# dRaniwal/RAJNI-ViT

Hardware: AMD Instinct MI355X
Metric: images/sec ViT-B/16@224 with README schedule (higher is better)
Workload: dtype bf16

## Files before the change

### rajni-vit_amd/csrc/gemm.hip

```cpp
#include <stdlib.h>
#include <type_traits>
#include "common.h"

namespace {

enum { EPI_BIAS = 0, EPI_GELU = 1, EPI_RESID = 2, EPI_PATCH = 3,
       EPI_GELU8 = 4 };
enum { ALOAD_PLAIN = 0, ALOAD_PATCH = 1 };

struct GemmParams {
  const void* X; long lda;
  const void* W; long ldw;
  const float* wscale;
  const float* xscale;
  const float* yscale;
  const float* bias;
  const float* gamma;
  const void* R; long ldr;
  const int* ridx; int r_np, r_nsrc;
  void* Y; long ldc;
  int M, N, K;
  int tiles_n, total_tiles;
  int nblk;
  int cin, S, log2ps, gw, npatch;
// ... 78 lines not shown
template <bool NT>
__device__ __forceinline__ void store_u4(void* ptr, const uint4& v) {
  if constexpr (NT) __builtin_nontemporal_store(u32x4{v.x, v.y, v.z, v.w}, reinterpret_cast<u32x4*>(ptr));
  else *reinterpret_cast<uint4*>(ptr) = v;
}

template <int EPI, bool SF32, typename A>
__device__ __forceinline__ void epilogue_row(const GemmParams& p, int m, int nbA, int nbB, float* v, const float* gam) {
  long orow = m;
  const bool full = nbB + 8 <= p.N;
  if (EPI == EPI_GELU) {
#pragma unroll
    for (int j = 0; j < 16; j += 4) {
      f32x2 a = f32x2{v[j], v[j + 1]}, b = f32x2{v[j + 2], v[j + 3]};
      gelu_pk4(a, b);
      v[j] = a[0]; v[j + 1] = a[1]; v[j + 2] = b[0]; v[j + 3] = b[1];
    }
  } else if (EPI == EPI_RESID) {
    long rrow = m;
    if (p.ridx != nullptr) {
      const int b = m / p.r_np;
      rrow = (long)b * p.r_nsrc + p.ridx[m];
    }
    const long rbase = rrow * p.ldr;
    if (full) {
      float rf[16];
      load8s<SF32, A>(p.R, rbase + nbA, rf);
      load8s<SF32, A>(p.R, rbase + nbB, rf + 8);
#pragma unroll
      for (int j = 0; j < 16; ++j) v[j] = fmaf(gam[j], v[j], rf[j]);
    } else {
#pragma unroll
      for (int j = 0; j < 16; ++j) {
        const int n = (j < 8 ? nbA : nbB - 8) + j;
        if (n < p.N) v[j] = fmaf(gam[j], v[j], load1<SF32, A>(p.R, rbase + n));
      }
    }
  } else if (EPI == EPI_PATCH) {
    const int b = m / p.npatch, pp = m - b * p.npatch;
    orow = (long)b * (p.npatch + p.nprefix) + p.nprefix + pp;
    const A* pr = reinterpret_cast<const A*>(p.pos) + (long)(pp + p.pos_off) * p.ldc;
    if (full) {
      float pf[16];
      unpack8<A>(*reinterpret_cast<const uint4*>(pr + nbA), pf);
      unpack8<A>(*reinterpret_cast<const uint4*>(pr + nbB), pf + 8);
#pragma unroll
      for (int j = 0; j < 16; ++j) v[j] += pf[j];
    } else {
#pragma unroll
      for (int j = 0; j < 16; ++j) {
        const int n = (j < 8 ? nbA : nbB - 8) + j;
        if (n < p.N) v[j] += ld1(pr + n);
      }
    }
  }
  constexpr bool OUT32 = SF32 && (EPI == EPI_RESID || EPI == EPI_PATCH);
  const long ybase = orow * p.ldc;
  if (full) {
    store8s<OUT32, A>(p.Y, ybase + nbA, v);
    store8s<OUT32, A>(p.Y, ybase + nbB, v + 8);
  } else {
#pragma unroll
    for (int j = 0; j < 16; ++j) {
      const int n = (j < 8 ? nbA : nbB - 8) + j;
      if (n < p.N) store1<OUT32, A>(p.Y, ybase + n, v[j]);
    }
  }
}

constexpr bool nat_order(int epi, bool sf32) { return sf32 && (epi == EPI_RESID || epi == EPI_PATCH); }

enum { MAP_NAT = 1, MAP_SEC = 2, MAP_F8 = 3 };
constexpr int col_map(int epi, bool sf32) { return epi == EPI_GELU8 ? MAP_F8 : nat_order(epi, sf32) ? MAP_NAT : MAP_SEC; }

#ifndef RAJNI_TSTORE
#define RAJNI_TSTORE 1
#endif
#ifndef RAJNI_F8W_LINES
#define RAJNI_F8W_LINES 1
#endif
constexpr bool resid_nat(int epi, bool sf32) { return nat_order(epi, sf32) && epi == EPI_RESID; }
constexpr bool epi_rowmajor(int epi, bool sf32, int mi) { return resid_nat(epi, sf32) && mi <= 4; }
constexpr bool epi_rowmajor_wide(int epi, bool sf32, int mi, bool w8) { return resid_nat(epi, sf32) && mi > 4 && !w8; }
constexpr bool epi_tstore(int epi) { return RAJNI_TSTORE && (epi == EPI_BIAS || epi == EPI_GELU); }
constexpr int stream_scratch_bytes(int epi, bool sf32, int mi, bool w8) {
  return (epi_rowmajor(epi, sf32, mi) || epi_rowmajor_wide(epi, sf32, mi, w8) || epi_tstore(epi)) ? 2048 : 0;
}
constexpr int f8_scratch_bytes(int epi, bool sf32) {
  return (resid_nat(epi, sf32) || epi == EPI_BIAS) ? 2048 : 0;
}
constexpr int f8w_scratch_bytes(int epi) { return (epi == EPI_BIAS && RAJNI_F8W_LINES) ? 4096 : 0; }
constexpr int LDS_MAX_BYTES = 160 * 1024;

template <int MAP>
__device__ __forceinline__ int out_col(int n0w, int g, int j) {
  const int ni = j >> 2, rg = j & 3;
  return MAP == MAP_NAT ? n0w + 16 * ni + 4 * g + rg
       : MAP == MAP_F8 ? n0w + 16 * g + 4 * ni + rg : n0w + 32 * (ni >> 1) + 8 * g + 4 * (ni & 1) + rg;
}
template <int MAP>
__device__ __forceinline__ int w_frag_row(int l15, int ni) {
  return MAP == MAP_NAT ? ni * 16 + l15
       : MAP == MAP_F8 ? 16 * (l15 >> 2) + 4 * ni + (l15 & 3) : 32 * (ni >> 1) + 8 * (l15 >> 2) + 4 * (ni & 1) + (l15 & 3);
}
template <int MAP>
__device__ __forceinline__ int w_key(int row) {
  return MAP == MAP_NAT ? (row >> 1) & 7
       : MAP == MAP_F8 ? ((row >> 4) & 3) * 2 + ((row >> 1) & 1) : ((row >> 3) & 3) * 2 + ((row >> 1) & 1);
}

template <int MAP>
__device__ __forceinline__ int w_key8(int row) {
  return MAP == MAP_NAT ? (row >> 2) & 3 : (row >> 3) & 3;
}
__device__ __forceinline__ bf16x8 fp8x8_to_bf16(uint2 raw) {
  const bf16x2 a = __builtin_amdgcn_cvt_scalef32_pk_bf16_fp8(raw.x, 1.0f, false);
  const bf16x2 b = __builtin_amdgcn_cvt_scalef32_pk_bf16_fp8(raw.x, 1.0f, true);
  const bf16x2 c = __builtin_amdgcn_cvt_scalef32_pk_bf16_fp8(raw.y, 1.0f, false);
  const bf16x2 d = __builtin_amdgcn_cvt_scalef32_pk_bf16_fp8(raw.y, 1.0f, true);
  return bf16x8{a[0], a[1], b[0], b[1], c[0], c[1], d[0], d[1]};
}
typedef __attribute__((ext_vector_type(4))) __bf16 fp8x8_raw;
template <bool W8> struct WFragT { typedef bf16x8 type; };
template <> struct WFragT<true> { typedef fp8x8_raw type; };
__device__ __forceinline__ bf16x8 w_frag_bf16(const bf16x8& f) { return f; }
__device__ __forceinline__ bf16x8 w_frag_bf16(const fp8x8_raw& f) { return fp8x8_to_bf16(__builtin_bit_cast(uint2, f)); }

template <int EPI, typename A>
__device__ __forceinline__ void epilogue_row_nat(const GemmParams& p, int m, int n0w, int g, float* v, const float* gam) {
  long orow = m, rrow = m;
  int pp = 0;
  if (EPI == EPI_RESID && p.ridx != nullptr) {
    const int b = m / p.r_np;
    rrow = (long)b * p.r_nsrc + p.ridx[m];
  }
  if (EPI == EPI_PATCH) {
    const int b = m / p.npatch;
    pp = m - b * p.npatch;
    orow = (long)b * (p.npatch + p.nprefix) + p.nprefix + pp;
  }
  const float* R = reinterpret_cast<const float*>(p.R);
  const A* P = reinterpret_cast<const A*>(p.pos);
  float* Y = reinterpret_cast<float*>(p.Y);
#pragma unroll
  for (int ni = 0; ni < 4; ++ni) {
    const int c = n0w + 16 * ni + 4 * g;
    float* vv = v + 4 * ni;
    if (c + 4 <= p.N) {
      if (EPI == EPI_RESID) {
        const float4 r = *reinterpret_cast<const float4*>(R + rrow * p.ldr + c);
        vv[0] = fmaf(gam[4 * ni + 0], vv[0], r.x); vv[1] = fmaf(gam[4 * ni + 1], vv[1], r.y);
        vv[2] = fmaf(gam[4 * ni + 2], vv[2], r.z); vv[3] = fmaf(gam[4 * ni + 3], vv[3], r.w);
      } else {
        const uint2 q = *reinterpret_cast<const uint2*>(P + (long)(pp + p.pos_off) * p.ldc + c);
        vv[0] += lo16<A>(q.x); vv[1] += hi16<A>(q.x); vv[2] += lo16<A>(q.y); vv[3] += hi16<A>(q.y);
      }
      *reinterpret_cast<float4*>(Y + orow * p.ldc + c) = make_float4(vv[0], vv[1], vv[2], vv[3]);
    } else {
#pragma unroll
      for (int e = 0; e < 4; ++e)
        if (c + e < p.N) {
          float o = vv[e];
          if (EPI == EPI_RESID) o = fmaf(gam[4 * ni + e], o, R[rrow * p.ldr + c + e]);
          else o += ld1(P + (long)(pp + p.pos_off) * p.ldc + c + e);
          Y[orow * p.ldc + c + e] = o;
          vv[e] = o;
// ... 48 lines not shown
                                               int l15, int g) {
  pre.valid = false;
  if constexpr (nat_order(EPI, SF32) && EPI == EPI_RESID && MI <= 4) {
    if (n0w + 64 <= p.N && m_base + MI * 16 <= p.M) {
      const float* R = reinterpret_cast<const float*>(p.R);
#pragma unroll
      for (int mi = 0; mi < MI; ++mi) {
        const int m = m_base + mi * 16 + l15;
        long rrow = m;
        if (p.ridx != nullptr) rrow = (long)(m / p.r_np) * p.r_nsrc + p.ridx[m];
#pragma unroll
        for (int ni = 0; ni < 4; ++ni)
          pre.r[mi][ni] = *reinterpret_cast<const float4*>(R + rrow * p.ldr + n0w + 16 * ni + 4 * g);
      }
      pre.valid = true;
    }
  }
}

constexpr int stores_acc_layout(bool nat, int mi) { return (nat ? 4 : 2) * mi; }
constexpr int stores_rowmajor(int mi) { return 2 * 2 * mi; }
constexpr int stores_tstore(int mi) { return 2 * mi; }
constexpr int tile_stores(int epi, bool sf32, int mi, bool rowmajor, bool tstore) {
  int n = stores_acc_layout(nat_order(epi, sf32), mi);
  if (rowmajor && stores_rowmajor(mi) < n) n = stores_rowmajor(mi);
  if (tstore && stores_tstore(mi) < n) n = stores_tstore(mi);
  return n;
}

template <typename A, int EPI, bool SF32, int MI, bool W8 = false>
__device__ __forceinline__ void epilogue_tile(const GemmParams& p, f32x4 (&acc)[4][MI], int m_base, int n0w,
                                              int l15, int g, ResidPrefetch<MI>& pre, int m_lo = 0,
                                              bool interior = false, char* scratch = nullptr) {
  constexpr int MAP = col_map(EPI, SF32);
  constexpr bool NAT = MAP == MAP_NAT;
  if constexpr (NAT && EPI == EPI_RESID && MI <= 4) {
    if (scratch != nullptr && pre.valid) {
      int lane = g * 16 + l15;
      asm volatile("" : "+v"(lane));
      const int rr = lane >> 3, cc = lane & 7;
      float bias[2][4], gam[2][4], wsc[2][W8 ? 4 : 1];
#pragma unroll
      for (int hc = 0; hc < 2; ++hc) {
        const int n = n0w + 32 * hc + 4 * cc;
        const float4 bq = p.bias != nullptr ? *reinterpret_cast<const float4*>(p.bias + n) : make_float4(0.f, 0.f, 0.f, 0.f);
        const float4 gq = p.gamma != nullptr ? *reinterpret_cast<const float4*>(p.gamma + n) : make_float4(1.f, 1.f, 1.f, 1.f);
        bias[hc][0] = bq.x; bias[hc][1] = bq.y; bias[hc][2] = bq.z; bias[hc][3] = bq.w;
        gam[hc][0] = gq.x; gam[hc][1] = gq.y; gam[hc][2] = gq.z; gam[hc][3] = gq.w;
        if constexpr (W8) {
          const float4 wq = *reinterpret_cast<const float4*>(p.wscale + n);
          wsc[hc][0] = wq.x; wsc[hc][1] = wq.y; wsc[hc][2] = wq.z; wsc[hc][3] = wq.w;
        }
      }
      __builtin_amdgcn_s_waitcnt(0x0F70);
      float* Y = reinterpret_cast<float*>(p.Y) + n0w + 4 * cc;
#pragma unroll
      for (int mi = 0; mi < MI; ++mi)
#pragma unroll
        for (int hc = 0; hc < 2; ++hc) {
#pragma unroll
          for (int q = 0; q < 2; ++q) {
            const int slot = (4 * q + g) ^ (l15 & 7);
            *reinterpret_cast<bf16x8*>(scratch + l15 * 128 + slot * 16) = __builtin_bit_cast(bf16x8, acc[2 * hc + q][mi]);
          }
          __builtin_amdgcn_fence(__ATOMIC_RELEASE, "wavefront");
          __builtin_amdgcn_wave_barrier();
#pragma unroll
          for (int j = 0; j < 2; ++j) {
            const int row = 8 * j + rr, slot = cc ^ (row & 7);
            const f32x4 a = __builtin_bit_cast(f32x4, *reinterpret_cast<const bf16x8*>(scratch + row * 128 + slot * 16));
            const float4 r = pre.r[mi][2 * hc + j];
            float4 o;
            o.x = fmaf(gam[hc][0], W8 ? fmaf(a[0], wsc[hc][0], bias[hc][0]) : a[0] + bias[hc][0], r.x);
            o.y = fmaf(gam[hc][1], W8 ? fmaf(a[1], wsc[hc][1], bias[hc][1]) : a[1] + bias[hc][1], r.y);
            o.z = fmaf(gam[hc][2], W8 ? fmaf(a[2], wsc[hc][2], bias[hc][2]) : a[2] + bias[hc][2], r.z);
            o.w = fmaf(gam[hc][3], W8 ? fmaf(a[3], wsc[hc][3], bias[hc][3]) : a[3] + bias[hc][3], r.w);
            *reinterpret_cast<float4*>(Y + (long)(m_base + mi * 16 + row) * p.ldc + 32 * hc) = o;
          }
          __builtin_amdgcn_wave_barrier();
        }
      return;
    }
  }
  if constexpr (NAT && EPI == EPI_RESID && MI > 4 && !W8) {
    if (scratch != nullptr && interior && p.ridx == nullptr) {
      int lane = g * 16 + l15;
      asm volatile("" : "+v"(lane));
      const int rr = lane >> 3, cc = lane & 7;
      float bias[2][4], gam[2][4];
#pragma unroll
      for (int hc = 0; hc < 2; ++hc) {
        const int n = n0w + 32 * hc + 4 * cc;
        const float4 bq = p.bias != nullptr ? *reinterpret_cast<const float4*>(p.bias + n) : make_float4(0.f, 0.f, 0.f, 0.f);
        const float4 gq = p.gamma != nullptr ? *reinterpret_cast<const float4*>(p.gamma + n) : make_float4(1.f, 1.f, 1.f, 1.f);
        bias[hc][0] = bq.x; bias[hc][1] = bq.y; bias[hc][2] = bq.z; bias[hc][3] = bq.w;
        gam[hc][0] = gq.x; gam[hc][1] = gq.y; gam[hc][2] = gq.z; gam[hc][3] = gq.w;
      }
      const float* R = reinterpret_cast<const float*>(p.R) + n0w + 4 * cc;
      float* Y = reinterpret_cast<float*>(p.Y) + n0w + 4 * cc;
#pragma unroll
      for (int mi = 0; mi < MI; ++mi) {
        float4 r[4];
#pragma unroll
        for (int j = 0; j < 2; ++j) {
          const long ro = (long)(m_base + mi * 16 + 8 * j + rr) * p.ldr;
          r[j] = *reinterpret_cast<const float4*>(R + ro);
          r[2 + j] = *reinterpret_cast<const float4*>(R + ro + 32);
        }
#pragma unroll
        for (int hc = 0; hc < 2; ++hc) {
#pragma unroll
          for (int q = 0; q < 2; ++q) {
            const int slot = (4 * q + g) ^ (l15 & 7);
            *reinterpret_cast<bf16x8*>(scratch + l15 * 128 + slot * 16) = __builtin_bit_cast(bf16x8, acc[2 * hc + q][mi]);
          }
          __builtin_amdgcn_fence(__ATOMIC_RELEASE, "wavefront");
          __builtin_amdgcn_wave_barrier();
#pragma unroll
          for (int j = 0; j < 2; ++j) {
            const int row = 8 * j + rr, slot = cc ^ (row & 7);
            const f32x4 a = __builtin_bit_cast(f32x4, *reinterpret_cast<const bf16x8*>(scratch + row * 128 + slot * 16));
            float4 o;
            o.x = fmaf(gam[hc][0], a[0] + bias[hc][0], r[2 * hc + j].x);
            o.y = fmaf(gam[hc][1], a[1] + bias[hc][1], r[2 * hc + j].y);
            o.z = fmaf(gam[hc][2], a[2] + bias[hc][2], r[2 * hc + j].z);
            o.w = fmaf(gam[hc][3], a[3] + bias[hc][3], r[2 * hc + j].w);
            *reinterpret_cast<float4*>(Y + (long)(m_base + mi * 16 + row) * p.ldc + 32 * hc) = o;
          }
          __builtin_amdgcn_wave_barrier();
        }
      }
      __builtin_amdgcn_s_waitcnt(0x0F70);
      return;
    }
  }
  if constexpr (MAP == MAP_SEC && (EPI == EPI_BIAS || EPI == EPI_GELU)) {
    if (interior) {
      const int ca = n0w + 8 * g, cb = ca + 32;
      float bs[16], ws[16];
#pragma unroll
      for (int j = 0; j < 16; ++j) { bs[j] = 0.f; ws[j] = 1.f; }
      if (p.bias != nullptr) {
        load8<float>(p.bias + ca, bs);
        load8<float>(p.bias + cb, bs + 8);
      }
      if constexpr (W8) {
        load8<float>(p.wscale + ca, ws);
        load8<float>(p.wscale + cb, ws + 8);
      }
      __builtin_amdgcn_s_waitcnt(0x0F70);
      A* Y = reinterpret_cast<A*>(p.Y);
#pragma unroll
      for (int mi = 0; mi < MI; ++mi) {
        float v[16];
#pragma unroll
        for (int j = 0; j < 16; ++j) {
          const int ni = j >> 2, rg = j & 3, o = (ni >> 1) * 8 + (ni & 1) * 4 + rg;
          v[o] = W8 ? fmaf(acc[ni][mi][rg], ws[o], bs[o]) : acc[ni][mi][rg] + bs[o];
        }
        if (EPI == EPI_GELU) {
#pragma unroll
          for (int j = 0; j < 16; j += 4) {
            f32x2 a = f32x2{v[j], v[j + 1]}, b = f32x2{v[j + 2], v[j + 3]};
            gelu_pk4(a, b);
            v[j] = a[0]; v[j + 1] = a[1]; v[j + 2] = b[0]; v[j + 3] = b[1];
          }
        }
        if (scratch != nullptr) {
          int lane = g * 16 + l15;
          asm volatile("" : "+v"(lane));
          const int rr = lane >> 3, cc = lane & 7;
          const int key = l15 & 7;
          *reinterpret_cast<bf16x8*>(scratch + l15 * 128 + ((g ^ key) << 4)) = __builtin_bit_cast(bf16x8, pack8<A>(v));
          *reinterpret_cast<bf16x8*>(scratch + l15 * 128 + (((4 + g) ^ key) << 4)) = __builtin_bit_cast(bf16x8, pack8<A>(v + 8));
          __builtin_amdgcn_fence(__ATOMIC_RELEASE, "wavefront");
          __builtin_amdgcn_wave_barrier();
#pragma unroll
          for (int j = 0; j < 2; ++j) {
            const int row = 8 * j + rr;
            const uint4 q = __builtin_bit_cast(uint4, *reinterpret_cast<const bf16x8*>(scratch + row * 128 + ((cc ^ (row & 7)) << 4)));
            store_u4<RAJNI_FC1_NT && EPI == EPI_GELU>(Y + (long)(m_base + mi * 16 + row) * p.ldc + n0w + 8 * cc, q);
          }
          __builtin_amdgcn_wave_barrier();
        } else {
          A* row = Y + (long)(m_base + mi * 16 + l15) * p.ldc;
          store_u4<RAJNI_FC1_NT && EPI == EPI_GELU>(row + ca, pack8<A>(v));
          store_u4<RAJNI_FC1_NT && EPI == EPI_GELU>(row + cb, pack8<A>(v + 8));
        }
      }
      return;
    }
  }
  float bias[16], gam[16];
#pragma unroll
  for (int j = 0; j < 16; ++j) {
    const int n = out_col<MAP>(n0w, g, j);
    bias[j] = (p.bias != nullptr && n < p.N) ? p.bias[n] : 0.f;
    gam[j] = (EPI == EPI_RESID && p.gamma != nullptr && n < p.N) ? p.gamma[n] : 1.f;
  }
  float wsc[W8 ? 16 : 1];
  if constexpr (W8) {
#pragma unroll
    for (int j = 0; j < 16; ++j) {
      const int n = out_col<MAP>(n0w, g, j);
      wsc[j] = n < p.N ? p.wscale[n] : 0.f;
    }
  }
  __builtin_amdgcn_s_waitcnt(0x0F70);
  auto sb = [&](float a, int j) { return W8 ? fmaf(a, wsc[W8 ? j : 0], bias[j]) : a + bias[j]; };
  if constexpr (NAT && EPI == EPI_RESID && MI <= 4) {
    if (pre.valid) {
      float* Y = reinterpret_cast<float*>(p.Y);
#pragma unroll
      for (int mi = 0; mi < MI; ++mi) {
#pragma unroll
        for (int ni = 0; ni < 4; ++ni) {
          float4 o;
          o.x = fmaf(gam[4 * ni + 0], sb(acc[ni][mi][0], 4 * ni + 0), pre.r[mi][ni].x);
          o.y = fmaf(gam[4 * ni + 1], sb(acc[ni][mi][1], 4 * ni + 1), pre.r[mi][ni].y);
          o.z = fmaf(gam[4 * ni + 2], sb(acc[ni][mi][2], 4 * ni + 2), pre.r[mi][ni].z);
          o.w = fmaf(gam[4 * ni + 3], sb(acc[ni][mi][3], 4 * ni + 3), pre.r[mi][ni].w);
          *reinterpret_cast<float4*>(Y + (long)(m_base + mi * 16 + l15) * p.ldc + n0w + 16 * ni + 4 * g) = o;
        }
      }
      return;
    }
  }
#pragma unroll
  for (int mi = 0; mi < MI; ++mi) {
    const int m = m_base + mi * 16 + l15;
    if (m >= p.M || m < m_lo) continue;
    float v[16];
#pragma unroll
    for (int ni = 0; ni < 4; ++ni)
#pragma unroll
      for (int rg = 0; rg < 4; ++rg) v[ni * 4 + rg] = sb(acc[ni][mi][rg], ni * 4 + rg);
    if (NAT) epilogue_row_nat<EPI, A>(p, m, n0w, g, v, gam);
    else epilogue_row<EPI, SF32, A>(p, m, n0w + 8 * g, n0w + 32 + 8 * g, v, gam);
  }
}
__device__ __forceinline__ int xcd_tile_of(int v, int total) {
  const int q = total >> 3, r = total & 7, xcd = v & 7, loc = v >> 3;
  return (xcd < r ? xcd * (q + 1) : r * (q + 1) + (xcd - r) * q) + loc;
}
__device__ __forceinline__ int xcd_tile(int total) { return xcd_tile_of(blockIdx.x, total); }

template <int ALOAD, typename ET = bf16_t>
struct XSource {
  static constexpr int CH = 16 / (int)sizeof(ET);
  const ET* base;
  int kofs;
  __device__ __forceinline__ void init(const GemmParams& p, int m, int chunk) {
    const ET* X = reinterpret_cast<const ET*>(p.X);
    if (ALOAD == ALOAD_PLAIN) {
      base = X + (long)m * p.lda + chunk * CH;
      kofs = 0;
    } else {
      const int b = m / p.npatch, pp = m - b * p.npatch;
      const int py = pp / p.gw, px = pp - py * p.gw;
      base = X + ((long)b * p.cin * p.S + (py << p.log2ps)) * p.S + (px << p.log2ps);
      kofs = chunk * CH;
    }
  }
  __device__ __forceinline__ const ET* at(const GemmParams& p, int k0) const {
    if (ALOAD == ALOAD_PLAIN) return base + k0;
    const int k = k0 + kofs, ps2 = 2 * p.log2ps;
    const int ch = k >> ps2, rem = k & ((1 << ps2) - 1);
    const int ky = rem >> p.log2ps, kx = rem & ((1 << p.log2ps) - 1);
    return base + ((long)ch * p.S + ky) * p.S + kx;
  }
};

#define RAJNI_GEMM_NBLK_BYTES (1600 * 1024)
namespace wide {
constexpr int BM = 256, BK = 64;
constexpr int X_BYTES = BM * BK * 2;
__device__ __forceinline__ int key_x(int row) { return (row >> 1) & 7; }

template <int WN_, int NS_, bool W8_ = false, int NW_ = 8> struct Cfg {
  static constexpr int BN = WN_ * 64;
  static constexpr int WB = W8_ ? 1 : 2;
  static constexpr int W_BYTES = BN * BK * WB;
  static constexpr int STAGE_BYTES = X_BYTES + W_BYTES;
  static constexpr int LDS_BYTES = NS_ * STAGE_BYTES;
  static constexpr int XP = X_BYTES / 1024 / NW_;
  static constexpr int PW = W_BYTES / 1024 / NW_;
  static constexpr int PIECES = XP + PW;
  static constexpr int NPW = PW < (W8_ ? 2 : 4) ? PW : (W8_ ? 2 : 4);
};
template <int EPI, bool SF32, int WN, int MI, int NS, bool W8>
constexpr int lds_bytes() { return Cfg<WN, NS, W8>::LDS_BYTES + 8 * stream_scratch_bytes(EPI, SF32, MI, W8); }

__host__ __device__ constexpr int dma_first(int g, int pieces, int groups) { return g * pieces / groups; }
__host__ __device__ constexpr int rd_first(int g, int mi, int ni) { return g + g * ni / mi; }
template <int G, int MI, bool DMA, int PIECES, int NI = 4>
__device__ __forceinline__ void sched_half() {
  if constexpr (G < MI) {
    __builtin_amdgcn_sched_group_barrier(0x008, NI, 0);
    if constexpr (rd_first(G + 1, MI, NI) - rd_first(G, MI, NI) > 0)
      __builtin_amdgcn_sched_group_barrier(0x100, rd_first(G + 1, MI, NI) - rd_first(G, MI, NI), 0);
    if constexpr (DMA) {
      constexpr int nd = dma_first(G + 1, PIECES, MI) - dma_first(G, PIECES, MI);
      if constexpr (nd > 0) __builtin_amdgcn_sched_group_barrier(0x020, nd, 0);
    }
    sched_half<G + 1, MI, DMA, PIECES, NI>();
  }
}
template <int N> __device__ __forceinline__ void wait_step() {
  static_assert(N >= 0 && N < 64, "vmcnt is a 6-bit counter");
  asm volatile("s_waitcnt vmcnt(%0) lgkmcnt(0)" :: "n"(N) : "memory");
}

template <int EPI, int ALOAD, bool SF32, int WM, int WN, int MI, int NS, bool W8 = false, int TAG = 0, typename A = bf16_t>
__global__ void __launch_bounds__(WM * WN * 64, 2) gemm_bf16_tn_stream(const GemmParams p) {
  using C = Cfg<WN, NS, W8, WM * WN>;
  constexpr int NI = 4;
  using WFrag = typename WFragT<W8>::type;
  constexpr int MAP = col_map(EPI, SF32);
  static_assert(WM * WN == 8 && WM * MI * 16 == BM, "8 waves covering 256 rows");
  extern __shared__ __attribute__((aligned(16))) char smem[];
  const int tid = threadIdx.x, lane = tid & 63;
  const int wave = __builtin_amdgcn_readfirstlane(tid >> 6);
  constexpr bool ROWMAJOR = epi_rowmajor(EPI, SF32, MI);
  constexpr int SCRATCH = stream_scratch_bytes(EPI, SF32, MI, W8);
  static_assert(lds_bytes<EPI, SF32, WN, MI, NS, W8>() <= LDS_MAX_BYTES, "stages + epilogue scratch exceed the workgroup's LDS");

  auto tile_m0 = [&](int tm_) { return tm_ * BM + BM > p.M ? p.M - BM : tm_ * BM; };
  const int tiles_m = p.total_tiles / p.tiles_n;
  auto tile_mn = [&](int t, int& tm_, int& tn_) {
    if (p.nblk >= p.tiles_n) { tm_ = t / p.tiles_n; tn_ = t - tm_ * p.tiles_n; return; }
    const int per = p.nblk * tiles_m, blk = t / per, r = t - blk * per;
    const int left = p.tiles_n - blk * p.nblk, nb = left < p.nblk ? left : p.nblk;
    const int rr = r / nb;
    tm_ = rr; tn_ = blk * p.nblk + (r - rr * nb);
  };
  XSource<ALOAD> xs[ALOAD == ALOAD_PLAIN ? 1 : C::XP];
  const char* xp[2];
  const char* ws[C::NPW];
  auto point_at = [&](int tile) {
    int tm, tn;
    tile_mn(tile, tm, tn);
    const int r_in = lane >> 3, pch = lane & 7;
    if constexpr (ALOAD == ALOAD_PLAIN) {
#pragma unroll
      for (int i = 0; i < 2; ++i) {
        const int row = (wave * C::XP + i) * 8 + r_in;
        xp[i] = reinterpret_cast<const char*>(p.X) + ((long)(tile_m0(tm) + row) * p.lda + (pch ^ key_x(row)) * 8) * 2;
      }
    } else {
#pragma unroll
      for (int i = 0; i < C::XP; ++i) {
        const int row = (wave * C::XP + i) * 8 + r_in;
        int m = tm * BM + row;
        if (m > p.M - 1) m = p.M - 1;
        xs[i].init(p, m, pch ^ key_x(row));
      }
    }
#pragma unroll
    for (int i = 0; i < C::NPW; ++i) {
      if constexpr (W8) {
        const int row = (wave * C::PW + i) * 16 + (lane >> 2);
        ws[i] = reinterpret_cast<const char*>(p.W) + (long)(tn * C::BN + row) * p.ldw + (((lane & 3) ^ w_key8<MAP>(row)) << 4);
      } else {
        const int row = (wave * C::PW + i) * 8 + r_in;
        ws[i] = reinterpret_cast<const char*>(p.W) + ((long)(tn * C::BN + row) * p.ldw + (pch ^ w_key<MAP>(row)) * 8) * 2;
      }
    }
  };
  auto advance = [&](int from, int to) {
    if constexpr (ALOAD == ALOAD_PLAIN) {
      int tm0, tn0, tm1, tn1;
      tile_mn(from, tm0, tn0);
      tile_mn(to, tm1, tn1);
      const long dx = (long)(tile_m0(tm1) - tile_m0(tm0)) * p.lda * 2;
      const long dw = (long)(tn1 - tn0) * C::BN * p.ldw * C::WB;
      xp[0] += dx; xp[1] += dx;
#pragma unroll
      for (int i = 0; i < C::NPW; ++i) ws[i] += dw;
    } else {
      point_at(to);
    }
  };
  auto dma_piece = [&](int q, int k0, char* dx) {
    if (q < C::XP) {
      if constexpr (ALOAD == ALOAD_PLAIN)
        __builtin_amdgcn_global_load_lds(GLB_PTR(xp[q & 1] + ((long)(q >> 1) * 16 * p.lda + k0) * 2),
                                         LDS_PTR(dx + (wave * C::XP + q) * 1024), 16, 0, 0);
      else
        __builtin_amdgcn_global_load_lds(GLB_PTR(xs[q].at(p, k0)), LDS_PTR(dx + (wave * C::XP + q) * 1024), 16, 0, 0);
    } else {
      const int i = q - C::XP;
      if constexpr (C::PW <= C::NPW)
        __builtin_amdgcn_global_load_lds(GLB_PTR(ws[i] + k0 * C::WB), LDS_PTR(dx + X_BYTES + (wave * C::PW + i) * 1024), 16, 0, 0);
      else
        __builtin_amdgcn_global_load_lds(GLB_PTR(ws[i % C::NPW] + ((long)(i / C::NPW) * 32 * p.ldw + k0) * C::WB),
                                         LDS_PTR(dx + X_BYTES + (wave * C::PW + i) * 1024), 16, 0, 0);
    }
  };
  auto stage = [&](int kt, int st) {
#pragma unroll
    for (int q = 0; q < C::PIECES; ++q) dma_piece(q, kt * BK, smem + st * C::STAGE_BYTES);
  };

  const int wm = wave / WN, wn = wave % WN;
  const int l15 = lane & 15, g = lane >> 4;
  const int xr0 = wm * (MI * 16) + l15;
  const int wr0 = wn * 64 + w_frag_row<MAP>(l15, 0);
  auto w_ni_off = [](int ni) { return (w_frag_row<MAP>(0, ni) - w_frag_row<MAP>(0, 0)) * (64 * C::WB); };
  int xo[2], wo[2];
#pragma unroll
  for (int ks = 0; ks < 2; ++ks) {
    xo[ks] = xr0 * 128 + (((ks * 4 + g) ^ key_x(xr0)) << 4);
    if constexpr (W8)
      wo[ks] = X_BYTES + wr0 * 64 + ((((ks * 4 + g) >> 1) ^ w_key8<MAP>(wr0)) << 4) + ((g & 1) << 3);
    else
      wo[ks] = X_BYTES + wr0 * 128 + (((ks * 4 + g) ^ w_key<MAP>(wr0)) << 4);
  }

  f32x4 acc[4][MI];

  auto half = [&](auto dma_c, auto read_c, bf16x8 (&xc)[MI], WFrag (&wc)[NI], bf16x8 (&xn)[MI], WFrag (&wn_)[NI],
                  int rst, int rks, int dkt, int dst) {
    constexpr bool DMA = decltype(dma_c)::value;
    constexpr bool READ = decltype(read_c)::value;
    const char* sb = smem + rst * C::STAGE_BYTES;
    char* dx = smem + dst * C::STAGE_BYTES;
    const int k0 = dkt * BK;
    bf16x8 wv[NI];
#pragma unroll
    for (int ni = 0; ni < NI; ++ni) wv[ni] = w_frag_bf16(wc[ni]);
#pragma unroll
    for (int mi = 0; mi < MI; ++mi) {
#pragma unroll
      for (int ni = 0; ni < NI; ++ni)
        acc[ni][mi] = mfma_16x16x32<A>(wv[ni], xc[mi], acc[ni][mi]);
      if constexpr (READ) {
        xn[mi] = *reinterpret_cast<const bf16x8*>(sb + xo[rks] + mi * 2048);
#pragma unroll
        for (int wi = mi * NI / MI; wi < (mi + 1) * NI / MI; ++wi)
          wn_[wi] = *reinterpret_cast<const WFrag*>(sb + wo[rks] + w_ni_off(wi));
      }
      if constexpr (DMA) {
#pragma unroll
        for (int q = dma_first(mi, C::PIECES, MI); q < dma_first(mi + 1, C::PIECES, MI); ++q) dma_piece(q, k0, dx);
      }
    }
    if constexpr (READ) sched_half<0, MI, DMA, C::PIECES, NI>();
  };
  using T = std::true_type; using F = std::false_type;
  const int nk = p.K / BK;
  int v = blockIdx.x;
  int tile = xcd_tile_of(v, p.total_tiles);
  bf16x8 xa[MI], xb[MI];
  WFrag wa[NI], wb[NI];
  if constexpr (EPI == EPI_RESID) {
    if (p.stagger > 0 && ((blockIdx.x >> 3) & 1))
      for (int i = 0; i < p.stagger; ++i) __builtin_amdgcn_s_sleep(127);
  }

  constexpr int WBASE = (NS - 2) * C::PIECES;
  auto interior = [&](int t) {
    int tm_, tn_;
    tile_mn(t, tm_, tn_);
    return tm_ * BM + BM <= p.M && tn_ * C::BN + C::BN <= p.N;
  };
  ResidPrefetch<MI> pre;
  point_at(tile);
#pragma unroll
  for (int j = 0; j < NS; ++j) stage(j, j);
  wait_step<((NS - 1) * C::PIECES > 8) ? 0 : (NS - 1) * C::PIECES>();
  __builtin_amdgcn_s_barrier();
  asm volatile("" ::: "memory");
#pragma unroll
  for (int i = 0; i < NI; ++i) wa[i] = *reinterpret_cast<const WFrag*>(smem + wo[0] + w_ni_off(i));
#pragma unroll
  for (int i = 0; i < MI; ++i) xa[i] = *reinterpret_cast<const bf16x8*>(smem + xo[0] + i * 2048);
  int st = 0;
  constexpr int NSTORE_ALL = tile_stores(EPI, SF32, MI, ROWMAJOR || epi_rowmajor_wide(EPI, SF32, MI, W8), epi_tstore(EPI));
  constexpr int NSTORE = NSTORE_ALL < 48 ? NSTORE_ALL : 48;
  bool prev_full = false;

  while (true) {
#ifdef RAJNI_GEMM_STAMPS
    const unsigned long long ts0 = __builtin_amdgcn_s_memtime();
#endif
    int tm, tn;
    tile_mn(tile, tm, tn);
    const int m0 = ALOAD == ALOAD_PLAIN ? tile_m0(tm) : tm * BM, n0 = tn * C::BN;
    const int m_lo = tm * BM;
    const bool inter = interior(tile);
    const int vn = v + gridDim.x;
    const bool more = vn < p.total_tiles;
    pre.valid = false;
#pragma unroll
    for (int a = 0; a < 4; ++a)
#pragma unroll
      for (int b = 0; b < MI; ++b) acc[a][b] = f32x4{0.f, 0.f, 0.f, 0.f};

    auto kstep = [&](int kt) {
      if (kt == nk - NS && more) advance(tile, xcd_tile_of(vn, p.total_tiles));
      const int dkt = kt + NS < nk ? kt + NS : kt + NS - nk;
      const int st1 = st + 1 == NS ? 0 : st + 1;
      if (kt == nk - 1 && inter) {
        if constexpr (ROWMAJOR) prefetch_resid_rowmajor<MI>(p, pre, m0 + wm * (MI * 16), n0 + wn * 64, lane);
        else prefetch_resid<EPI, SF32, MI>(p, pre, m0 + wm * (MI * 16), n0 + wn * 64, l15, g);
      }
      half(F{}, T{}, xa, wa, xb, wb, st, 1, 0, 0);
      if (NSTORE > 0 && kt == 0 && prev_full) wait_step<WBASE + NSTORE>();
      else wait_step<WBASE>();
      __builtin_amdgcn_s_barrier();
      asm volatile("" ::: "memory");
      half(T{}, T{}, xb, wb, xa, wa, st1, 0, dkt, st);
      st = st1;
    };
    for (int kt = 0; kt < nk; ++kt) kstep(kt);
#ifdef RAJNI_GEMM_STAMPS
    asm volatile("" :: "v"(acc[0][0][0]), "v"(acc[3][MI - 1][3]));
    const unsigned long long ts2 = __builtin_amdgcn_s_memtime();
#endif

    epilogue_tile<A, EPI, SF32, MI, W8>(p, acc, m0 + wm * (MI * 16), n0 + wn * 64, l15, g, pre, m_lo, inter,
                                     SCRATCH > 0 ? smem + C::LDS_BYTES + wave * SCRATCH : nullptr);
#ifdef RAJNI_GEMM_STAMPS
    if (p.stamps != nullptr && wave == 0) {
      const unsigned long long ts3 = __builtin_amdgcn_s_memtime();
      if (lane == 0) {
        unsigned long long* o = p.stamps + (size_t)tile * 4;
        o[0] = ts0; o[1] = ts0; o[2] = ts2; o[3] = ts3;
      }
    }
#endif
    prev_full = inter;
    if (!more) break;
    v = vn;
    tile = xcd_tile_of(v, p.total_tiles);
  }
  asm volatile("s_waitcnt vmcnt(0)" ::: "memory");
}
}

namespace small {
constexpr int BM = 128, BN = 128, BK = 64;
constexpr int TILE_BYTES = BM * BK * 2;
constexpr int STAGE_BYTES = 2 * TILE_BYTES;
constexpr int LDS_BYTES = 2 * STAGE_BYTES;
__device__ __forceinline__ int key_x(int row) { return (row >> 1) & 7; }
__device__ __forceinline__ int key_w(int row) { return ((row >> 4) & 3) * 2 + ((row >> 1) & 1); }

template <int EPI, int ALOAD, bool SF32, bool W8 = false, typename A = bf16_t>
__global__ void __launch_bounds__(256, 2) gemm_bf16_tn_128x128(const GemmParams p) {
  constexpr int MAP = col_map(EPI, SF32);
  constexpr int PW = W8 ? 2 : 4;
  using WFrag = typename WFragT<W8>::type;
  extern __shared__ __attribute__((aligned(16))) char smem[];
  const int tid = threadIdx.x, lane = tid & 63;
  const int wave = __builtin_amdgcn_readfirstlane(tid >> 6);
  const int t = xcd_tile(p.total_tiles);
  const int tm = t / p.tiles_n, tn = t - tm * p.tiles_n;
  const int m0 = tm * BM, n0 = tn * BN;

  const int r_in = lane >> 3, pch = lane & 7;
  XSource<ALOAD> xs[4];
  const char* ws[PW];
#pragma unroll
  for (int i = 0; i < 4; ++i) {
    const int row = (wave * 4 + i) * 8 + r_in;
    int m = m0 + row;
    if (m > p.M - 1) m = p.M - 1;
    xs[i].init(p, m, pch ^ key_x(row));
  }
#pragma unroll
  for (int i = 0; i < PW; ++i) {
    if constexpr (W8) {
      const int row = (wave * PW + i) * 16 + (lane >> 2);
      ws[i] = reinterpret_cast<const char*>(p.W) + (long)(n0 + row) * p.ldw + (((lane & 3) ^ w_key8<MAP>(row)) << 4);
    } else {
      const int row = (wave * PW + i) * 8 + r_in;
      ws[i] = reinterpret_cast<const char*>(p.W) + ((long)(n0 + row) * p.ldw + (pch ^ w_key<MAP>(row)) * 8) * 2;
    }
  }
  auto stage = [&](int kt, int buf) {
    char* sx = smem + buf * STAGE_BYTES;
    char* sw = sx + TILE_BYTES;
    const int k0 = kt * BK;
#pragma unroll
    for (int i = 0; i < 4; ++i)
      __builtin_amdgcn_global_load_lds(GLB_PTR(xs[i].at(p, k0)), LDS_PTR(sx + (wave * 4 + i) * 1024), 16, 0, 0);
#pragma unroll
    for (int i = 0; i < PW; ++i)
      __builtin_amdgcn_global_load_lds(GLB_PTR(ws[i] + k0 * (W8 ? 1 : 2)), LDS_PTR(sw + (wave * PW + i) * 1024), 16, 0, 0);
  };

  const int wm = wave >> 1, wn = wave & 1;
  const int l15 = lane & 15, g = lane >> 4;
  int xoff[4], xkey[4], woff[4], wkey[4];
#pragma unroll
  for (int i = 0; i < 4; ++i) {
    const int xr = wm * 64 + i * 16 + l15;
    xoff[i] = xr * 128; xkey[i] = key_x(xr);
    const int wr = wn * 64 + w_frag_row<MAP>(l15, i);
    woff[i] = wr * (W8 ? 64 : 128); wkey[i] = W8 ? w_key8<MAP>(wr) : w_key<MAP>(wr);
  }

  f32x4 acc[4][4];
#pragma unroll
  for (int a = 0; a < 4; ++a)
#pragma unroll
    for (int b = 0; b < 4; ++b) acc[a][b] = f32x4{0.f, 0.f, 0.f, 0.f};

  const int nk = p.K / BK;
  ResidPrefetch<4> pre;
  pre.valid = false;
  stage(0, 0);
  for (int kt = 0; kt < nk; ++kt) {
    asm volatile("s_waitcnt vmcnt(0)" ::: "memory");
    __syncthreads();
    if (kt + 1 < nk) stage(kt + 1, (kt + 1) & 1);
    else prefetch_resid<EPI, SF32, 4>(p, pre, m0 + wm * 64, n0 + wn * 64, l15, g);
// ... 568 lines not shown
```

Measured before the change: 30590.

## Stage residual tiles into LDS via DMA during the last k-steps of the wide resid GEMM

For the wide residual-epilogue GEMM variant, the last two k-steps are peeled. While they run, residual rows are loaded straight into freed LDS stage slots with global_load_lds, and the epilogue then reads them from LDS. The epilogue also refills slots and issues the next tile's operand DMA part-way through, so the residual read and the next tile's loads overlap with compute and stores. This adds complex vmcnt/lgkmcnt bookkeeping and slot-reuse hazards, and keeps a fallback path for non-interior tiles.

```diff
diff --git a/rajni-vit_amd/csrc/gemm.hip b/rajni-vit_amd/csrc/gemm.hip
--- a/rajni-vit_amd/csrc/gemm.hip
+++ b/rajni-vit_amd/csrc/gemm.hip
@@ -398,58 +398,6 @@
       return;
     }
   }
-  if constexpr (NAT && EPI == EPI_RESID && MI > 4 && !W8) {
-    if (scratch != nullptr && interior && p.ridx == nullptr) {
-      int lane = g * 16 + l15;
-      asm volatile("" : "+v"(lane));
-      const int rr = lane >> 3, cc = lane & 7;
-      float bias[2][4], gam[2][4];
-#pragma unroll
-      for (int hc = 0; hc < 2; ++hc) {
-        const int n = n0w + 32 * hc + 4 * cc;
-        const float4 bq = p.bias != nullptr ? *reinterpret_cast<const float4*>(p.bias + n) : make_float4(0.f, 0.f, 0.f, 0.f);
-        const float4 gq = p.gamma != nullptr ? *reinterpret_cast<const float4*>(p.gamma + n) : make_float4(1.f, 1.f, 1.f, 1.f);
-        bias[hc][0] = bq.x; bias[hc][1] = bq.y; bias[hc][2] = bq.z; bias[hc][3] = bq.w;
-        gam[hc][0] = gq.x; gam[hc][1] = gq.y; gam[hc][2] = gq.z; gam[hc][3] = gq.w;
-      }
-      const float* R = reinterpret_cast<const float*>(p.R) + n0w + 4 * cc;
-      float* Y = reinterpret_cast<float*>(p.Y) + n0w + 4 * cc;
-#pragma unroll
-      for (int mi = 0; mi < MI; ++mi) {
-        float4 r[4];
-#pragma unroll
-        for (int j = 0; j < 2; ++j) {
-          const long ro = (long)(m_base + mi * 16 + 8 * j + rr) * p.ldr;
-          r[j] = *reinterpret_cast<const float4*>(R + ro);
-          r[2 + j] = *reinterpret_cast<const float4*>(R + ro + 32);
-        }
-#pragma unroll
-        for (int hc = 0; hc < 2; ++hc) {
-#pragma unroll
-          for (int q = 0; q < 2; ++q) {
-            const int slot = (4 * q + g) ^ (l15 & 7);
-            *reinterpret_cast<bf16x8*>(scratch + l15 * 128 + slot * 16) = __builtin_bit_cast(bf16x8, acc[2 * hc + q][mi]);
-          }
-          __builtin_amdgcn_fence(__ATOMIC_RELEASE, "wavefront");
-          __builtin_amdgcn_wave_barrier();
-#pragma unroll
-          for (int j = 0; j < 2; ++j) {
-            const int row = 8 * j + rr, slot = cc ^ (row & 7);
-            const f32x4 a = __builtin_bit_cast(f32x4, *reinterpret_cast<const bf16x8*>(scratch + row * 128 + slot * 16));
-            float4 o;
-            o.x = fmaf(gam[hc][0], a[0] + bias[hc][0], r[2 * hc + j].x);
-            o.y = fmaf(gam[hc][1], a[1] + bias[hc][1], r[2 * hc + j].y);
-            o.z = fmaf(gam[hc][2], a[2] + bias[hc][2], r[2 * hc + j].z);
-            o.w = fmaf(gam[hc][3], a[3] + bias[hc][3], r[2 * hc + j].w);
-            *reinterpret_cast<float4*>(Y + (long)(m_base + mi * 16 + row) * p.ldc + 32 * hc) = o;
-          }
-          __builtin_amdgcn_wave_barrier();
-        }
-      }
-      __builtin_amdgcn_s_waitcnt(0x0F70);
-      return;
-    }
-  }
   if constexpr (MAP == MAP_SEC && (EPI == EPI_BIAS || EPI == EPI_GELU)) {
     if (interior) {
       const int ca = n0w + 8 * g, cb = ca + 32;
@@ -555,6 +503,76 @@
     else epilogue_row<EPI, SF32, A>(p, m, n0w + 8 * g, n0w + 32 + 8 * g, v, gam);
   }
 }
+__device__ __forceinline__ int lane_now() {
+  unsigned all = ~0u;
+  asm volatile("" : "+s"(all));
+  return (int)__builtin_amdgcn_mbcnt_hi(all, __builtin_amdgcn_mbcnt_lo(all, 0u));
+}
+constexpr int WIDE_LDS_STORES_AFTER_DMA = 4;
+template <int N> __device__ __forceinline__ void wait_vm() {
+  static_assert(N >= 0 && N < 64, "vmcnt is a 6-bit counter");
+  asm volatile("s_waitcnt vmcnt(%0)" :: "n"(N) : "memory");
+}
+__device__ const float WIDE_LDS_ZEROS[4] = {0.f, 0.f, 0.f, 0.f}, WIDE_LDS_ONES[4] = {1.f, 1.f, 1.f, 1.f};
+typedef __attribute__((address_space(1))) f32x4 GLB_F32X4;
+__device__ __forceinline__ unsigned resid_lane_offset(const GemmParams& p, int lane) {
+  return ((unsigned)(lane >> 3) * (unsigned)p.ldr + 4u * (unsigned)(lane & 7)) * 4u;
+}
+__device__ __forceinline__ void land_resid_piece(const GemmParams& p, unsigned lane_off, int m_base, int n0w, int grp, int pc, char* slot) {
+  const char* base = reinterpret_cast<const char*>(p.R) + ((long)(m_base + grp * 16 + (pc & 1) * 8) * p.ldr + n0w + (pc >> 1) * 32) * 4;
+  __builtin_amdgcn_global_load_lds(GLB_PTR(base + (unsigned long)lane_off), LDS_PTR(slot + pc * 1024), 16, 0, 0);
+}
+template <typename SlotFn, typename RefillFn>
+__device__ __forceinline__ void epilogue_wide_lds(const GemmParams& p, f32x4 (&acc)[4][8], int m_base, int n0w,
+                                                  const float (&bias)[2][4], const float (&gam)[2][4], char* scratch,
+                                                  SlotFn&& slot, RefillFn&& refill) {
+  const int lane = lane_now();
+  const int l15 = lane & 15, g = lane >> 4;
+  const int rr = lane >> 3, cc = lane & 7;
+  const unsigned ylo = ((unsigned)rr * (unsigned)p.ldc + 4u * (unsigned)cc) * 4u;
+#pragma unroll
+  for (int mi = 0; mi < 8; ++mi) {
+    if (mi == 0) wait_vm<12>();
+    else if (mi == 1) wait_vm<16>();
+    else if (mi == 2) wait_vm<20>();
+    else if (mi == 3) wait_vm<24>();
+    else wait_vm<28>();
+    const char* sl = slot(mi & 3) + lane * 16;
+    f32x4 r[4];
+#pragma unroll
+    for (int pc = 0; pc < 4; ++pc) r[pc] = __builtin_bit_cast(f32x4, *reinterpret_cast<const bf16x8*>(sl + pc * 1024));
+#pragma unroll
+    for (int hc = 0; hc < 2; ++hc) {
+#pragma unroll
+      for (int q = 0; q < 2; ++q) {
+        const int sw = (4 * q + g) ^ (l15 & 7);
+        *reinterpret_cast<bf16x8*>(scratch + l15 * 128 + sw * 16) = __builtin_bit_cast(bf16x8, acc[2 * hc + q][mi]);
+      }
+      __builtin_amdgcn_fence(__ATOMIC_RELEASE, "wavefront");
+      __builtin_amdgcn_wave_barrier();
+      f32x4 a[2];
+#pragma unroll
+      for (int j = 0; j < 2; ++j) {
+        const int row = 8 * j + rr, sw = cc ^ (row & 7);
+        a[j] = __builtin_bit_cast(f32x4, *reinterpret_cast<const bf16x8*>(scratch + row * 128 + sw * 16));
+      }
+      if (hc == 0) {
+        asm volatile("s_waitcnt lgkmcnt(0)" ::: "memory");
+        refill(mi);
+      }
+#pragma unroll
+      for (int j = 0; j < 2; ++j) {
+        const f32x4 rv = r[2 * hc + j];
+        f32x4 o;
+#pragma unroll
+        for (int e = 0; e < 4; ++e) o[e] = fmaf(gam[hc][e], a[j][e] + bias[hc][e], rv[e]);
+        char* yb = reinterpret_cast<char*>(p.Y) + ((long)(m_base + mi * 16 + 8 * j) * p.ldc + n0w + 32 * hc) * 4;
+        *(GLB_F32X4*)GLB_PTR(yb + (unsigned long)ylo) = o;
+      }
+      __builtin_amdgcn_wave_barrier();
+    }
+  }
+}
 __device__ __forceinline__ int xcd_tile_of(int v, int total) {
   const int q = total >> 3, r = total & 7, xcd = v & 7, loc = v >> 3;
   return (xcd < r ? xcd * (q + 1) : r * (q + 1) + (xcd - r) * q) + loc;
@@ -638,6 +656,8 @@
   const int tid = threadIdx.x, lane = tid & 63;
   const int wave = __builtin_amdgcn_readfirstlane(tid >> 6);
   constexpr bool ROWMAJOR = epi_rowmajor(EPI, SF32, MI);
+  constexpr bool LAND = epi_rowmajor_wide(EPI, SF32, MI, W8);
+  static_assert(!LAND || (NS == 2 && C::XP == 4 && C::PW == 4 && ALOAD == ALOAD_PLAIN), "a slot = the 4 pieces one wave stages of one operand");
   constexpr int SCRATCH = stream_scratch_bytes(EPI, SF32, MI, W8);
   static_assert(lds_bytes<EPI, SF32, WN, MI, NS, W8>() <= LDS_MAX_BYTES, "stages + epilogue scratch exceed the workgroup's LDS");
 
@@ -793,12 +813,22 @@
   for (int i = 0; i < MI; ++i) xa[i] = *reinterpret_cast<const bf16x8*>(smem + xo[0] + i * 2048);
   int st = 0;
   constexpr int NSTORE_ALL = tile_stores(EPI, SF32, MI, ROWMAJOR || epi_rowmajor_wide(EPI, SF32, MI, W8), epi_tstore(EPI));
-  constexpr int NSTORE = NSTORE_ALL < 48 ? NSTORE_ALL : 48;
+  static_assert(!LAND || WIDE_LDS_STORES_AFTER_DMA <= NSTORE_ALL, "the landing epilogue's count must be the smallest of the paths'");
+  constexpr int NSTORE = LAND ? WIDE_LDS_STORES_AFTER_DMA : NSTORE_ALL < 48 ? NSTORE_ALL : 48;
   bool prev_full = false;
 
   while (true) {
 #ifdef RAJNI_GEMM_STAMPS
     const unsigned long long ts0 = __builtin_amdgcn_s_memtime();
+    auto stamp_tile = [&](unsigned long long t0, unsigned long long t2) {
+      if (p.stamps != nullptr && wave == 0) {
+        const unsigned long long ts3 = __builtin_amdgcn_s_memtime();
+        if (lane == 0) {
+          unsigned long long* o = p.stamps + (size_t)tile * 4;
+          o[0] = t0; o[1] = t0; o[2] = t2; o[3] = ts3;
+        }
+      }
+    };
 #endif
     int tm, tn;
     tile_mn(tile, tm, tn);
@@ -829,22 +859,155 @@
       half(T{}, T{}, xb, wb, xa, wa, st1, 0, dkt, st);
       st = st1;
     };
-    for (int kt = 0; kt < nk; ++kt) kstep(kt);
+    [[maybe_unused]] bool landed = false;
+    if constexpr (!LAND) {
+      for (int kt = 0; kt < nk; ++kt) kstep(kt);
+    } else {
+      landed = inter && p.ridx == nullptr && p.ldr < (1L << 26) && p.ldc < (1L << 26);
+      const int nk_main = landed ? nk - 2 : nk;
+      for (int kt = 0; kt < nk_main; ++kt) kstep(kt);
+    }
+    [[maybe_unused]] float lbias[2][4], lgam[2][4];
+    [[maybe_unused]] int st_a = 0;
+    if constexpr (LAND) {
+      if (landed) {
+        const int mw = m0 + wm * (MI * 16), nw = n0 + wn * 64;
+        st_a = st;
+        auto slot = [&](int s) { return smem + ((s >> 1) ? st_a ^ 1 : st_a) * C::STAGE_BYTES + (s & 1) * X_BYTES + wave * 4096; };
+        auto land_piece = [&](unsigned lo, int grp, int pc) { land_resid_piece(p, lo, mw, nw, grp, pc, slot(grp & 3)); };
+        auto half_land = [&](auto read_c, bf16x8 (&xc)[MI], WFrag (&wc)[NI], bf16x8 (&xn)[MI], WFrag (&wn_)[NI], int rst, int grp0) {
+          constexpr bool READ = decltype(read_c)::value;
+          const char* sb = smem + rst * C::STAGE_BYTES;
+          const unsigned lo = resid_lane_offset(p, lane_now());
+          bf16x8 wv[NI];
+#pragma unroll
+          for (int ni = 0; ni < NI; ++ni) wv[ni] = w_frag_bf16(wc[ni]);
+#pragma unroll
+          for (int mi = 0; mi < MI; ++mi) {
+#pragma unroll
+            for (int ni = 0; ni < NI; ++ni)
+              acc[ni][mi] = mfma_16x16x32<A>(wv[ni], xc[mi], acc[ni][mi]);
+            if constexpr (READ) {
+              xn[mi] = *reinterpret_cast<const bf16x8*>(sb + xo[0] + mi * 2048);
+#pragma unroll
+              for (int wi = mi * NI / MI; wi < (mi + 1) * NI / MI; ++wi)
+                wn_[wi] = *reinterpret_cast<const WFrag*>(sb + wo[0] + w_ni_off(wi));
+            }
+            land_piece(lo, grp0 + (mi >> 2), mi & 3);
+          }
+          if constexpr (READ) {
+            sched_half<0, MI, true, C::PIECES, NI>();
+          } else {
+#pragma unroll
+            for (int mi = 0; mi < MI; ++mi) {
+              __builtin_amdgcn_sched_group_barrier(0x008, NI, 0);
+              __builtin_amdgcn_sched_group_barrier(0x020, 1, 0);
+            }
+          }
+        };
+        half(F{}, T{}, xa, wa, xb, wb, st, 1, 0, 0);
+        wait_step<WBASE>();
+        __builtin_amdgcn_s_barrier();
+        asm volatile("" ::: "memory");
+        half_land(T{}, xb, wb, xa, wa, st ^ 1, 0);
+        st ^= 1;
+        half(F{}, T{}, xa, wa, xb, wb, st, 1, 0, 0);
+        asm volatile("s_waitcnt lgkmcnt(0)" ::: "memory");
+        __builtin_amdgcn_s_barrier();
+        asm volatile("" ::: "memory");
+        {
+          const bool hb = p.bias != nullptr, hg = p.gamma != nullptr;
+          const char* bsrc = hb ? reinterpret_cast<const char*>(p.bias + nw) : reinterpret_cast<const char*>(WIDE_LDS_ZEROS);
+          const char* gsrc = hg ? reinterpret_cast<const char*>(p.gamma + nw) : reinterpret_cast<const char*>(WIDE_LDS_ONES);
+          const unsigned lo = 16u * (unsigned)(lane_now() & 7);
+          const unsigned blo = hb ? lo : 0u, glo = hg ? lo : 0u, bhi = hb ? 128u : 0u, ghi = hg ? 128u : 0u;
+#pragma unroll
+          for (int hc = 0; hc < 2; ++hc) {
+            const f32x4 bq = *(const GLB_F32X4*)GLB_PTR(bsrc + (unsigned long)(blo + bhi * hc));
+            const f32x4 gq = *(const GLB_F32X4*)GLB_PTR(gsrc + (unsigned long)(glo + ghi * hc));
+#pragma unroll
+            for (int e = 0; e < 4; ++e) {
+              lbias[hc][e] = bq[e];
+              lgam[hc][e] = gq[e];
+            }
+          }
+        }
+        half_land(F{}, xb, wb, xa, wa, 0, 2);
+        st ^= 1;
+      }
+    }
 #ifdef RAJNI_GEMM_STAMPS
     asm volatile("" :: "v"(acc[0][0][0]), "v"(acc[3][MI - 1][3]));
     const unsigned long long ts2 = __builtin_amdgcn_s_memtime();
 #endif
 
-    epilogue_tile<A, EPI, SF32, MI, W8>(p, acc, m0 + wm * (MI * 16), n0 + wn * 64, l15, g, pre, m_lo, inter,
-                                     SCRATCH > 0 ? smem + C::LDS_BYTES + wave * SCRATCH : nullptr);
+    if constexpr (LAND) {
+      if (landed) {
+        const int mw = m0 + wm * (MI * 16), nw = n0 + wn * 64;
+        auto slot = [&](int s) { return smem + ((s >> 1) ? st_a ^ 1 : st_a) * C::STAGE_BYTES + (s & 1) * X_BYTES + wave * 4096; };
+        auto refill = [&](int mi) {
+          if (mi < 4) {
+            const unsigned lo = resid_lane_offset(p, lane_now());
+#pragma unroll
+            for (int pc = 0; pc < 4; ++pc) land_resid_piece(p, lo, mw, nw, mi + 4, pc, slot(mi));
+          } else {
+            if (mi == 4) {
+              int ptm, ptn;
+              tile_mn(more ? xcd_tile_of(vn, p.total_tiles) : tile, ptm, ptn);
+              const int ln = lane_now(), r_in = ln >> 3, pch = ln & 7;
+#pragma unroll
+              for (int i = 0; i < 2; ++i) {
+                const int row = (wave * C::XP + i) * 8 + r_in;
+                xp[i] = reinterpret_cast<const char*>(p.X) + ((long)(tile_m0(ptm) + row) * p.lda + (pch ^ key_x(row)) * 8) * 2;
+              }
+#pragma unroll
+              for (int i = 0; i < C::NPW; ++i) {
+                const int row = (wave * C::PW + i) * 8 + r_in;
+                ws[i] = reinterpret_cast<const char*>(p.W) + ((long)(ptn * C::BN + row) * p.ldw + (pch ^ w_key<MAP>(row)) * 8) * 2;
+              }
+            }
+#pragma unroll
+            for (int q = 0; q < 4; ++q)
+              dma_piece(4 * (mi & 1) + q, ((mi >> 1) & 1) * BK, smem + ((mi & 2) ? st_a ^ 1 : st_a) * C::STAGE_BYTES);
+          }
+        };
+        epilogue_wide_lds(p, acc, mw, nw, lbias, lgam, smem + C::LDS_BYTES + wave * SCRATCH, slot, refill);
+        prev_full = true;
+        {
+          const int ln = lane_now(), rl15 = ln & 15, rg = ln >> 4;
+          const int rxr0 = wm * (MI * 16) + rl15, rwr0 = wn * 64 + w_frag_row<MAP>(rl15, 0);
+#pragma unroll
+          for (int ks = 0; ks < 2; ++ks) {
+            xo[ks] = rxr0 * 128 + (((ks * 4 + rg) ^ key_x(rxr0)) << 4);
+            wo[ks] = X_BYTES + rwr0 * 128 + (((ks * 4 + rg) ^ w_key<MAP>(rwr0)) << 4);
+          }
+        }
+        if (more) {
+          wait_step<WIDE_LDS_STORES_AFTER_DMA + 16>();
+          __builtin_amdgcn_s_barrier();
+          asm volatile("" ::: "memory");
+#pragma unroll
+          for (int i = 0; i < NI; ++i) wa[i] = *reinterpret_cast<const WFrag*>(smem + st * C::STAGE_BYTES + wo[0] + w_ni_off(i));
+#pragma unroll
+          for (int i = 0; i < MI; ++i) xa[i] = *reinterpret_cast<const bf16x8*>(smem + st * C::STAGE_BYTES + xo[0] + i * 2048);
+        }
 #ifdef RAJNI_GEMM_STAMPS
-    if (p.stamps != nullptr && wave == 0) {
-      const unsigned long long ts3 = __builtin_amdgcn_s_memtime();
-      if (lane == 0) {
-        unsigned long long* o = p.stamps + (size_t)tile * 4;
-        o[0] = ts0; o[1] = ts0; o[2] = ts2; o[3] = ts3;
-      }
-    }
+        stamp_tile(ts0, ts2);
+#endif
+        if (!more) break;
+        v = vn;
+        tile = xcd_tile_of(v, p.total_tiles);
+        continue;
+      } else {
+        epilogue_tile<A, EPI, SF32, MI, W8>(p, acc, m0 + wm * (MI * 16), n0 + wn * 64, l15, g, pre, m_lo, inter, nullptr);
+        __builtin_amdgcn_s_waitcnt(0x0F70);
+      }
+    } else {
+      epilogue_tile<A, EPI, SF32, MI, W8>(p, acc, m0 + wm * (MI * 16), n0 + wn * 64, l15, g, pre, m_lo, inter,
+                                       SCRATCH > 0 ? smem + C::LDS_BYTES + wave * SCRATCH : nullptr);
+    }
+#ifdef RAJNI_GEMM_STAMPS
+    stamp_tile(ts0, ts2);
 #endif
     prev_full = inter;
     if (!more) break;
```

Result: no change. 30380 (-0.7%).

## Software-pipeline residual loads in wide resid epilogue with windowed prefetch

Applied to the files above, without the earlier changes.

In the wide (MI>4) residual epilogue, residual rows are now prefetched in a sliding window of several mi-rows ahead, using scalar base pointers and 32-bit lane offsets, with a partial vmcnt wait instead of loading each row just before use. The goal is to hide global-load latency in the fp32 residual-add epilogue and cut per-element 64-bit address arithmetic. For this epilogue variant the persistent-tile loop also reloads the first A/W fragments from LDS after the epilogue. This raises register pressure because several rows of residual values stay live at once, and it adds an ldr/ldc size guard.

```diff
diff --git a/rajni-vit_amd/csrc/gemm.hip b/rajni-vit_amd/csrc/gemm.hip
--- a/rajni-vit_amd/csrc/gemm.hip
+++ b/rajni-vit_amd/csrc/gemm.hip
@@ -184,6 +184,9 @@
 constexpr bool resid_nat(int epi, bool sf32) { return nat_order(epi, sf32) && epi == EPI_RESID; }
 constexpr bool epi_rowmajor(int epi, bool sf32, int mi) { return resid_nat(epi, sf32) && mi <= 4; }
 constexpr bool epi_rowmajor_wide(int epi, bool sf32, int mi, bool w8) { return resid_nat(epi, sf32) && mi > 4 && !w8; }
+#ifndef RAJNI_WIDE_RESID_WINDOW
+#define RAJNI_WIDE_RESID_WINDOW 4
+#endif
 constexpr bool epi_tstore(int epi) { return RAJNI_TSTORE && (epi == EPI_BIAS || epi == EPI_GELU); }
 constexpr int stream_scratch_bytes(int epi, bool sf32, int mi, bool w8) {
   return (epi_rowmajor(epi, sf32, mi) || epi_rowmajor_wide(epi, sf32, mi, w8) || epi_tstore(epi)) ? 2048 : 0;
@@ -399,7 +402,7 @@
     }
   }
   if constexpr (NAT && EPI == EPI_RESID && MI > 4 && !W8) {
-    if (scratch != nullptr && interior && p.ridx == nullptr) {
+    if (scratch != nullptr && interior && p.ridx == nullptr && p.ldr < (1L << 24) && p.ldc < (1L << 24)) {
       int lane = g * 16 + l15;
       asm volatile("" : "+v"(lane));
       const int rr = lane >> 3, cc = lane & 7;
@@ -412,17 +415,31 @@
         bias[hc][0] = bq.x; bias[hc][1] = bq.y; bias[hc][2] = bq.z; bias[hc][3] = bq.w;
         gam[hc][0] = gq.x; gam[hc][1] = gq.y; gam[hc][2] = gq.z; gam[hc][3] = gq.w;
       }
-      const float* R = reinterpret_cast<const float*>(p.R) + n0w + 4 * cc;
-      float* Y = reinterpret_cast<float*>(p.Y) + n0w + 4 * cc;
+      __builtin_amdgcn_sched_barrier(0);
+      const unsigned ro = (unsigned)(rr * (int)p.ldr + 4 * cc) * 4u, yo = (unsigned)(rr * (int)p.ldc + 4 * cc) * 4u;
+      unsigned long R = reinterpret_cast<unsigned long>(reinterpret_cast<const float*>(p.R) + (long)m_base * p.ldr + n0w);
+      unsigned long Y = reinterpret_cast<unsigned long>(reinterpret_cast<float*>(p.Y) + (long)m_base * p.ldc + n0w);
+      const long rstep = 8 * p.ldr * 4, ystep = 8 * p.ldc * 4;
+      typedef __attribute__((address_space(1))) const f32x4* GlobalLd;
+      typedef __attribute__((address_space(1))) f32x4* GlobalSt;
+      f32x4 r[MI][4];
+      auto issue = [&](int mi) {
+#pragma unroll
+        for (int j = 0; j < 2; ++j) {
+          asm volatile("" : "+s"(R));
+          r[mi][j] = *(GlobalLd)(R + ro);
+          r[mi][2 + j] = ((GlobalLd)(R + ro))[8];
+          R += rstep;
+        }
+      };
+#pragma unroll
+      for (int mi = 0; mi < RAJNI_WIDE_RESID_WINDOW && mi < MI; ++mi) issue(mi);
+      constexpr int WINDOW_LOADS = 4 * (RAJNI_WIDE_RESID_WINDOW < MI ? RAJNI_WIDE_RESID_WINDOW : MI);
+      static_assert(WINDOW_LOADS < 64, "vmcnt is a 6-bit counter");
+      __builtin_amdgcn_s_waitcnt(0x0F70 | (WINDOW_LOADS & 15) | ((WINDOW_LOADS >> 4) << 14));
 #pragma unroll
       for (int mi = 0; mi < MI; ++mi) {
-        float4 r[4];
-#pragma unroll
-        for (int j = 0; j < 2; ++j) {
-          const long ro = (long)(m_base + mi * 16 + 8 * j + rr) * p.ldr;
-          r[j] = *reinterpret_cast<const float4*>(R + ro);
-          r[2 + j] = *reinterpret_cast<const float4*>(R + ro + 32);
-        }
+        __builtin_amdgcn_sched_barrier(0);
 #pragma unroll
         for (int hc = 0; hc < 2; ++hc) {
 #pragma unroll
@@ -436,17 +453,21 @@
           for (int j = 0; j < 2; ++j) {
             const int row = 8 * j + rr, slot = cc ^ (row & 7);
             const f32x4 a = __builtin_bit_cast(f32x4, *reinterpret_cast<const bf16x8*>(scratch + row * 128 + slot * 16));
-            float4 o;
-            o.x = fmaf(gam[hc][0], a[0] + bias[hc][0], r[2 * hc + j].x);
-            o.y = fmaf(gam[hc][1], a[1] + bias[hc][1], r[2 * hc + j].y);
-            o.z = fmaf(gam[hc][2], a[2] + bias[hc][2], r[2 * hc + j].z);
-            o.w = fmaf(gam[hc][3], a[3] + bias[hc][3], r[2 * hc + j].w);
-            *reinterpret_cast<float4*>(Y + (long)(m_base + mi * 16 + row) * p.ldc + 32 * hc) = o;
+            f32x4 o;
+            o.x = fmaf(gam[hc][0], a[0] + bias[hc][0], r[mi][2 * hc + j].x);
+            o.y = fmaf(gam[hc][1], a[1] + bias[hc][1], r[mi][2 * hc + j].y);
+            o.z = fmaf(gam[hc][2], a[2] + bias[hc][2], r[mi][2 * hc + j].z);
+            o.w = fmaf(gam[hc][3], a[3] + bias[hc][3], r[mi][2 * hc + j].w);
+            unsigned long yq = Y + j * ystep;
+            asm volatile("" : "+s"(yq));
+            ((GlobalSt)(yq + yo))[8 * hc] = o;
           }
           __builtin_amdgcn_wave_barrier();
         }
-      }
-      __builtin_amdgcn_s_waitcnt(0x0F70);
+        Y += 2 * ystep;
+        __builtin_amdgcn_sched_barrier(0);
+        if (mi + RAJNI_WIDE_RESID_WINDOW < MI) issue(mi + RAJNI_WIDE_RESID_WINDOW);
+      }
       return;
     }
   }
@@ -639,6 +660,7 @@
   const int wave = __builtin_amdgcn_readfirstlane(tid >> 6);
   constexpr bool ROWMAJOR = epi_rowmajor(EPI, SF32, MI);
   constexpr int SCRATCH = stream_scratch_bytes(EPI, SF32, MI, W8);
+  constexpr bool LATE_FRAGS = epi_rowmajor_wide(EPI, SF32, MI, W8);
   static_assert(lds_bytes<EPI, SF32, WN, MI, NS, W8>() <= LDS_MAX_BYTES, "stages + epilogue scratch exceed the workgroup's LDS");
 
   auto tile_m0 = [&](int tm_) { return tm_ * BM + BM > p.M ? p.M - BM : tm_ * BM; };
@@ -850,6 +872,13 @@
     if (!more) break;
     v = vn;
     tile = xcd_tile_of(v, p.total_tiles);
+    if constexpr (LATE_FRAGS) {
+      const char* sb = smem + st * C::STAGE_BYTES;
+#pragma unroll
+      for (int i = 0; i < NI; ++i) wa[i] = *reinterpret_cast<const WFrag*>(sb + wo[0] + w_ni_off(i));
+#pragma unroll
+      for (int i = 0; i < MI; ++i) xa[i] = *reinterpret_cast<const bf16x8*>(sb + xo[0] + i * 2048);
+    }
   }
   asm volatile("s_waitcnt vmcnt(0)" ::: "memory");
 }
```

Measured after the change: 30990 before, 31080 after, median of 6. About the same (+0.3%).
